# lyd405121/ti-raytrace

Measured on AMD Instinct MI355X. Metric: Mrays/s (primary+secondary) at 1024² 100k-tri, 1/2/4/8 GPU + HBM GB/s, higher is better.
Workload: dtype f32

## Files before the change

include/tirt.h:

```cpp
#ifndef TIRT_H
#define TIRT_H

#include <stdint.h>

#ifdef __cplusplus
extern "C" {
#endif

typedef struct tirt_ctx tirt_ctx;

#define TIRT_OK 0
#define TIRT_ERR_HIP (-1)
#define TIRT_ERR_ARG (-2)
#define TIRT_ERR_BUILD (-3)
#define TIRT_ERR_STACK (-4)

#define TIRT_TRAVERSE_ORDERED 0
#define TIRT_TRAVERSE_EXHAUSTIVE 1
#define TIRT_COUNT_NODES 2

typedef struct {
    uint64_t rays_closest;
    uint64_t rays_shadow;
    uint64_t box_closest;
// ... 92 lines not shown

int tirt_bvh_info(tirt_ctx *ctx, uint64_t out[4]);
int tirt_micro_gather_rate(tirt_ctx *ctx, uint64_t working_set_bytes, int iters, double *gbps_out);

int tirt_trace_timeline(tirt_ctx *ctx, uint64_t *out, int max_waves, int *n_waves);

int tirt_primary_beam_stats(tirt_ctx *ctx, uint64_t out[12]);

int tirt_stats(tirt_ctx *ctx, tirt_stats_t *out);
int tirt_stats_reset(tirt_ctx *ctx);

int tirt_kat_math(tirt_ctx *ctx, int fn, const float *x, const float *y, float *out, int n);
int tirt_kat_brdf(tirt_ctx *ctx, int which, const float *in, int in_stride, float *out, int out_stride, int n);
int tirt_kat_spec(tirt_ctx *ctx, int which, const float *in, int in_stride, float *out, int out_stride, int n);

typedef struct tirt_obj tirt_obj;
int tirt_obj_load(const char *path, tirt_obj **out);
void tirt_obj_free(tirt_obj *obj);
int tirt_obj_material_count(const tirt_obj *obj);
int tirt_obj_material_info(const tirt_obj *obj, int index, char *name, int name_cap, double *params, int *vertex_format,
                           int *is_default, long long *n_floats);
int tirt_obj_material_vertices(const tirt_obj *obj, int index, double *out, long long n_floats);

#ifdef __cplusplus
}
#endif
#endif
```

ti_raytrace_amd/_native.py:

```python
import ctypes as C
import os

import numpy as np

_HERE = os.path.dirname(os.path.abspath(__file__))
LIB_PATH = os.environ.get("TIRT_LIB_PATH") or os.path.join(_HERE, "csrc", "libtirt.so")

_f32p = np.ctypeslib.ndpointer(dtype=np.float32, flags="C_CONTIGUOUS")
_i32p = np.ctypeslib.ndpointer(dtype=np.int32, flags="C_CONTIGUOUS")


class TirtError(RuntimeError):
    pass


class TirtStackOverflow(TirtError):

    def __init__(self, msg, stats):
        TirtError.__init__(self, msg)
        self.stats = stats


ERR_STACK = -4

# ... 56 lines not shown
    "tirt_trace_shadow": (C.c_int, [_vp, _f32p, C.c_int, C.c_int, C.c_int, _f32p, _i32p, _vp]),
    "tirt_query_closest": (C.c_int, [_vp, _vp, C.c_int64, C.c_int64, C.c_int, C.c_int, _vp, _vp, _vp, C.c_int64, _vp, _vp]),
    "tirt_query_occluded": (C.c_int, [_vp, _vp, C.c_int64, C.c_int64, _vp, C.c_int64, C.c_float, C.c_int, C.c_int, _vp, _vp]),
    "tirt_comm_init": (C.c_int, [C.POINTER(_vp), C.c_int]),
    "tirt_film_reduce": (C.c_int, [C.POINTER(_vp), C.c_int, C.c_int]),
    "tirt_comm_destroy": (C.c_int, [C.POINTER(_vp), C.c_int]),
    "tirt_bvh_info": (C.c_int, [_vp, C.POINTER(C.c_uint64)]),
    "tirt_micro_gather_rate": (C.c_int, [_vp, C.c_uint64, C.c_int, C.POINTER(C.c_double)]),
    "tirt_trace_timeline": (C.c_int, [_vp, C.POINTER(C.c_uint64), C.c_int, C.POINTER(C.c_int)]),
    "tirt_primary_beam_stats": (C.c_int, [_vp, C.POINTER(C.c_uint64)]),
    "tirt_stats": (C.c_int, [_vp, C.POINTER(Stats)]),
    "tirt_stats_reset": (C.c_int, [_vp]),
    "tirt_kat_math": (C.c_int, [_vp, C.c_int, _f32p, _f32p, _f32p, C.c_int]),
    "tirt_kat_brdf": (C.c_int, [_vp, C.c_int, _f32p, C.c_int, _f32p, C.c_int, C.c_int]),
    "tirt_kat_spec": (C.c_int, [_vp, C.c_int, _f32p, C.c_int, _f32p, C.c_int, C.c_int]),
    "tirt_obj_load": (C.c_int, [C.c_char_p, C.POINTER(_vp)]),
    "tirt_obj_free": (None, [_vp]),
    "tirt_obj_material_count": (C.c_int, [_vp]),
    "tirt_obj_material_info": (C.c_int, [_vp, C.c_int, C.c_char_p, C.c_int, C.POINTER(C.c_double), C.POINTER(C.c_int),
                                         C.POINTER(C.c_int), C.POINTER(C.c_longlong)]),
    "tirt_obj_material_vertices": (C.c_int, [_vp, C.c_int, np.ctypeslib.ndpointer(dtype=np.float64, flags="C_CONTIGUOUS"), C.c_longlong]),
}

class SpectralTables(C.Structure):
    _fields_ = [("sensor", C.c_void_p), ("n_sensor", C.c_int), ("s_min", C.c_float), ("s_max", C.c_float), ("s_range", C.c_float),
                ("spd", C.c_void_p), ("spd_n", C.c_int * 4), ("spd_min", C.c_float * 4), ("spd_max", C.c_float * 4), ("spd_range", C.c_float * 4),
                ("tbl_scale", C.c_void_p), ("tbl_data", C.c_void_p), ("tbl_res", C.c_int),
                ("sky_cfg", C.c_void_p), ("sky_rad", C.c_void_p), ("sun_dir", C.c_float * 3)]


# ... 282 lines not shown

    def kat_math(self, fn, x, y=None):
        x = np.ascontiguousarray(x, np.float32)
        y = np.ascontiguousarray(y if y is not None else np.zeros_like(x), np.float32)
        out = np.zeros_like(x)
        check(lib().tirt_kat_math(self.handle, int(fn), x, y, out, x.size))
        return out

    def kat_brdf(self, which, inp, out_stride):
        inp = np.ascontiguousarray(inp, np.float32)
        n, stride = inp.shape
        out = np.zeros((n, out_stride), np.float32)
        check(lib().tirt_kat_brdf(self.handle, int(which), inp.reshape(-1), stride, out.reshape(-1), out_stride, n))
        return out

    def kat_spec(self, which, inp, out_stride):
        inp = np.ascontiguousarray(inp, np.float32)
        n, stride = inp.shape
        out = np.zeros((n, out_stride), np.float32)
        check(lib().tirt_kat_spec(self.handle, int(which), inp.reshape(-1), stride, out.reshape(-1), out_stride, n))
        return out


def device_count():
    v = C.c_int(0)
    check(lib().tirt_device_count(C.byref(v)))
    return v.value


class Communicator:
# ... 14 lines not shown
```

ti_raytrace_amd/csrc/tirt_api.hip:

```cpp
#include "tirt_internal.h"
#include "tirt_spectral.h"
#include <stddef.h>
#include <mutex>
#include <string.h>

namespace tirt {

static thread_local std::string g_error;
void set_error(const std::string &msg) { g_error = msg; }

SceneView scene_view(const tirt_ctx *c)
{
    SceneView s;
    s.vertex = c->vertex.as<float>(); s.primitive = c->primitive.as<int>(); s.material = c->material.as<float>();
    s.shape = c->shape.as<float>(); s.light = c->light.as<int>(); s.env = c->env.as<int>();
    s.mat_lrgb = c->mat_lrgb.as<float>(); s.shade_rec = c->shade_rec.as<float4>();
    s.n = c->n; s.light_count = c->light_count; s.env_w = c->env_w; s.env_h = c->env_h; s.env_power = c->env_power;
    return s;
}
BvhView bvh_view(const tirt_ctx *c)
{
    BvhView b;
    b.wnode = c->wnode.as<float4>(); b.tri = c->tri.as<float4>();
    b.cnode = c->cnode.as<uint4>(); b.top_count = c->wide_nodes + c->n_far_nodes < TR_TOP_SLOTS ? c->wide_nodes + c->n_far_nodes : TR_TOP_SLOTS; b.compact = c->compact.as<float>(); b.cparent = c->cparent.as<int>();
    for (int k = 0; k < 3; k++) { b.grid_min[k] = c->grid_min[k]; b.cell[k] = c->grid_cell[k]; b.inv_cell[k] = c->grid_inv_cell[k]; b.inv_extent[k] = c->grid_inv_extent[k]; }
    for (int k = 0; k < 3; k++) { b.root_min[k] = c->root_min[k]; b.root_max[k] = c->root_max[k]; }
    b.root_code = c->root_code;
    b.root_qcode = c->root_code;
    b.far_qcode = c->n_far_nodes ? c->wide_nodes : c->root_code;
    return b;
}
// ... 31 lines not shown
}
static int refresh_material_table(tirt_ctx *c)
{
    if (c->mat_lrgb.ensure(sizeof(float) * 3 * (size_t)c->nm)) return TIRT_ERR_HIP;
    hipLaunchKernelGGL(k_material_lrgb, dim3((c->nm + 63) / 64), dim3(64), 0, c->stream, c->material.as<float>(), c->nm, c->mat_lrgb.as<float>());
    return 0;
}

__global__ void k_shade_records(SceneView s, float4 *rec)
{
    const int i = blockIdx.x * blockDim.x + threadIdx.x;
    if (i >= s.n) return;
    const int *pr = s.primitive + (size_t)i * PRI_VEC;
    float4 *r = rec + (size_t)i * 8;
    const float mat = __int_as_float(pr[2]);
    if (pr[0] == PRIMITIVE_TRI) {
        const v3 v1 = vtx_pos(s, pr[1]), v2 = vtx_pos(s, pr[1] + 1), v3_ = vtx_pos(s, pr[1] + 2);
        const v3 n1 = vtx_nor(s, pr[1]), n2 = vtx_nor(s, pr[1] + 1), n3 = vtx_nor(s, pr[1] + 2);
        r[0] = make_float4(v1.x, v1.y, v1.z, mat); r[1] = make_float4(v2.x, v2.y, v2.z, __int_as_float(PRIMITIVE_TRI));
        r[2] = make_float4(v3_.x, v3_.y, v3_.z, 0.0f);
        r[3] = make_float4(n1.x, n1.y, n1.z, 0.0f); r[4] = make_float4(n2.x, n2.y, n2.z, 0.0f); r[5] = make_float4(n3.x, n3.y, n3.z, 0.0f);
    } else {
        const float *sh = s.shape + (size_t)pr[1] * SHA_VEC;
        r[0] = make_float4(sh[1], sh[2], sh[3], mat); r[1] = make_float4(sh[4], sh[0], 0.0f, __int_as_float(2));
        r[2] = r[3] = r[4] = r[5] = make_float4(0.0f, 0.0f, 0.0f, 0.0f);
    }
    r[6] = r[7] = make_float4(0.0f, 0.0f, 0.0f, 0.0f);
}
int ensure_shade_records(tirt_ctx *c)
{
    if (c->shade_rec_valid && c->shade_rec.p) return 0;
    if (c->shade_rec.ensure(sizeof(float4) * 8 * (size_t)c->n)) return TIRT_ERR_HIP;
    hipLaunchKernelGGL(k_shade_records, dim3((c->n + 255) / 256), dim3(256), 0, c->stream, scene_view(c), c->shade_rec.as<float4>());
    c->shade_rec_valid = true;
    return 0;
}

__global__ void k_total_area(SceneView s, int count, float *out)
{
    if (blockIdx.x == 0 && threadIdx.x == 0) {
        float a = 0.0f;
        for (int i = 0; i < count; i++) a += get_prim_area(s, s.light[i]);
        *out = a;
    }
}

__global__ void k_smooth_normal(SceneView s, int nv, const float *compact, const int *vertex_index, float *smooth)
{
    int i = blockIdx.x * blockDim.x + threadIdx.x;
// ... 116 lines not shown
        o[0] = schlick_fresnel(a[0]);
    } else if (which == 16) {
        float fb; v3 r = glass_sample_lambda(V(a[0], a[1], a[2]), V(a[3], a[4], a[5]), a[6], a[7], fb); o[0] = r.x; o[1] = r.y; o[2] = r.z; o[3] = fb;
    } else if (which == 17) {
        CameraView cv; for (int k = 0; k < 12; k++) cv.view_inv[k] = a[k];
        cv.eye[0] = cv.eye[1] = cv.eye[2] = 0.0f; cv.fx = a[16]; cv.fy = a[17]; cv.cx = a[18]; cv.cy = a[19];
        v3 r = camera_ray_direction(cv, (int)a[20], (int)a[21], a[22], a[23]); o[0] = r.x; o[1] = r.y; o[2] = r.z;
    } else if (which == 18) {
        const RayCtx r = make_ray(V(a[0], a[1], a[2]), V(a[3], a[4], a[5])); float tn;
        const int full = slabs(r, a[6], a[7], a[8], a[9], a[10], a[11], tn);
        o[0] = (float)full;
        o[1] = ray_has_parallel_axis(r) ? (float)full : (float)slabs_fast(r, a[6], a[7], a[8], a[9], a[10], a[11], tn);
    }
}

TD uint32_t mg_mix(uint32_t x) { x ^= x >> 16; x *= 0x7feb352du; x ^= x >> 15; x *= 0x846ca68bu; x ^= x >> 16; return x; }
__global__ __launch_bounds__(256) void k_micro_gather(const float4 *rec, uint32_t nrec, int iters, float *out)
{
    uint32_t s = mg_mix(blockIdx.x * 256 + threadIdx.x + 1);
    float acc = 0.0f;
    for (int it = 0; it < iters; it++) {
        s = mg_mix(s + it);
        const uint32_t idx = (uint32_t)(((unsigned long long)s * nrec) >> 32);
        const float4 *p = rec + (size_t)idx * 4;
        const float4 a = p[0], b = p[1], c = p[2], d = p[3];
        acc += a.x + b.y + c.z + d.w;
    }
    out[blockIdx.x * 256 + threadIdx.x] = acc;
}

// ... 55 lines not shown
    if (hipDeviceGetAttribute(&cus, hipDeviceAttributeMultiprocessorCount, device_id) == hipSuccess && cus > 0) {
        const int g = 5 * cus < 2048 ? 5 * cus : 2048;
        c->tr_grid = g; c->tr_grid_alone = g; c->cu_count = cus;
    } else (void)hipGetLastError();
    *out = c;
    return TIRT_OK;
}

void tirt_destroy(tirt_ctx *c)
{
    if (!c) return;
    if (c->comm) { tirt_ctx *one[1] = {c}; (void)tirt_comm_destroy(one, 1); }
    (void)hipSetDevice(c->device);
    (void)sync_all(c);
    drain_render_events(c);
    DevBuf *bufs[] = {&c->vertex, &c->primitive, &c->material, &c->shape, &c->light, &c->env, &c->mat_lrgb, &c->shade_rec, &c->morton_unsorted, &c->keys_a,
                      &c->keys_b, &c->vals_a, &c->vals_b, &c->hist, &c->morton_sorted, &c->bvh_node, &c->compact, &c->parent,
                      &c->flag, &c->subtree, &c->build_status, &c->leaf_compact, &c->wnode, &c->tri, &c->prim_slot, &c->cnode, &c->cparent, &c->csize, &c->wide_queue, &c->wide_levels, &c->sah_compact, &c->sah_csize, &c->sah_parent, &c->wide_dp, &c->sah_box, &c->sah_idx, &c->sah_tasks, &c->sah_counts, &c->hdr, &c->rgb,
                      &c->counters_mem, &c->spill, &c->trace_stage, &c->debug_mem, &c->query_mem, &c->dev_counters, &c->bdpt_px, &c->timeline, &c->pvb_set[0].count, &c->pvb_set[0].cand, &c->pvb_set[0].bound, &c->pvb_set[1].count, &c->pvb_set[1].cand, &c->pvb_set[1].bound, &c->pvb_stat, &c->pvb_tmp};
    for (DevBuf *b : bufs) b->release();
    for (auto &bl : c->bd) {
        DevBuf *bb[] = {&bl.items, &bl.state, &bl.rays, &bl.hits, &bl.qidx, &bl.ctr, &bl.rad};
        for (DevBuf *b : bb) b->release();
        if (bl.delta_done) (void)hipEventDestroy(bl.delta_done);
        if (bl.film_done) (void)hipEventDestroy(bl.film_done);
    }
    for (Lane &L : c->lanes) {
        DevBuf *lb[] = {&L.path_mem, &L.counters_mem, &L.spill};
        for (DevBuf *b : lb) b->release();
        if (L.film_done) (void)hipEventDestroy(L.film_done);
        if (L.stream) (void)hipStreamDestroy(L.stream);
// ... 105 lines not shown
        TIRT_REQUIRE(pr[2] >= 0 && pr[2] < nm, "tirt_scene_upload: material index out of range");
    }
    for (int i = 0; i < nl; i++) TIRT_REQUIRE(light[i] >= 0 && light[i] < n, "tirt_scene_upload: light index out of range");
    c->sphere_prims.clear();
    for (int i = 0; i < n; i++) {
        const int32_t *pr = primitive + (size_t)i * 3;
        if (pr[0] != PRIMITIVE_TRI && (int)shape[(size_t)pr[1] * 10] == SHAPE_SPHERE) c->sphere_prims.push_back(i);
    }
    hipStream_t st = c->stream;
    c->built = false;
    if (upload(c->vertex, vertex, sizeof(float) * 9 * (size_t)nv, st)) return TIRT_ERR_HIP;
    if (upload(c->primitive, primitive, sizeof(int) * 3 * (size_t)n, st)) return TIRT_ERR_HIP;
    if (upload(c->material, material, sizeof(float) * 10 * (size_t)nm, st)) return TIRT_ERR_HIP;
    if (upload(c->shape, shape, sizeof(float) * 10 * (size_t)ns, st)) return TIRT_ERR_HIP;
    if (upload(c->light, light, sizeof(int) * (size_t)nl, st)) return TIRT_ERR_HIP;
    c->nv = nv; c->n = n; c->nm = nm; c->ns = ns; c->nl = nl; c->light_count = light_count; c->shade_rec_valid = false;
    for (int k = 0; k < 3; k++) { c->bmin[k] = bmin[k]; c->bmax[k] = bmax[k]; }
    if (refresh_material_table(c)) return TIRT_ERR_HIP;
    if (!c->env.p) {
        int32_t z = 0;
        if (upload(c->env, &z, sizeof(int32_t), st)) return TIRT_ERR_HIP;
        c->env_w = 1; c->env_h = 1; c->env_power = 0.0f;
    }
    TIRT_HIP(hipStreamSynchronize(st));
    return TIRT_OK;
}

int tirt_material_upload(tirt_ctx *c, const float *material, int nm)
{
    CTX(c);
    if (sync_all(c)) return TIRT_ERR_HIP;
    TIRT_REQUIRE(material && nm == c->nm, "tirt_material_upload: material count differs from the uploaded scene");
    if (upload(c->material, material, sizeof(float) * 10 * (size_t)nm, c->stream)) return TIRT_ERR_HIP;
    if (refresh_material_table(c)) return TIRT_ERR_HIP;
    TIRT_HIP(hipStreamSynchronize(c->stream));
    return TIRT_OK;
}

int tirt_env_upload(tirt_ctx *c, const int32_t *rgb_packed, int w, int h, float power)
{
    CTX(c);
    if (sync_all(c)) return TIRT_ERR_HIP;
    TIRT_REQUIRE(rgb_packed && w >= 1 && h >= 1, "tirt_env_upload: bad image");
    if (upload(c->env, rgb_packed, sizeof(int32_t) * (size_t)w * h, c->stream)) return TIRT_ERR_HIP;
    c->env_w = w; c->env_h = h; c->env_power = power;
    TIRT_HIP(hipStreamSynchronize(c->stream));
    return TIRT_OK;
}

// ... 56 lines not shown
}

int tirt_process_normal(tirt_ctx *c, const int32_t *vertex_index)
{
    CTX(c);
    if (sync_all(c)) return TIRT_ERR_HIP;
    TIRT_REQUIRE(c->built && vertex_index, "tirt_process_normal: LBVH not built");
    if (c->nv == 0) return TIRT_OK;
    for (int i = 0; i < c->nv; i++) TIRT_REQUIRE(vertex_index[i] >= 0 && vertex_index[i] < c->n, "tirt_process_normal: vertex_index out of range");
    DevBuf vi, smooth;
    if (upload(vi, vertex_index, sizeof(int) * (size_t)c->nv, c->stream)) return TIRT_ERR_HIP;
    if (smooth.ensure(sizeof(float) * 3 * (size_t)c->nv)) { vi.release(); return TIRT_ERR_HIP; }
    const int B = 128, G = (c->nv + B - 1) / B;
    hipLaunchKernelGGL(k_smooth_normal, dim3(G), dim3(B), 0, c->stream, scene_view(c), c->nv, c->compact.as<float>(), vi.as<int>(), smooth.as<float>());
    hipLaunchKernelGGL(k_write_normal, dim3(G), dim3(B), 0, c->stream, c->vertex.as<float>(), c->nv, smooth.as<float>());
    c->shade_rec_valid = false;
    hipError_t e = hipStreamSynchronize(c->stream);
    vi.release(); smooth.release();
    TIRT_HIP(e);
    TIRT_HIP(hipGetLastError());
    return TIRT_OK;
}

int tirt_vertex_download(tirt_ctx *c, float *vertex)
{
    CTX(c);
    TIRT_REQUIRE(vertex, "tirt_vertex_download: null");
    TIRT_HIP(hipMemcpyAsync(vertex, c->vertex.p, sizeof(float) * 9 * (size_t)c->nv, hipMemcpyDeviceToHost, c->stream));
    TIRT_HIP(hipStreamSynchronize(c->stream));
    return TIRT_OK;
}
// ... 325 lines not shown
    TIRT_REQUIRE(in_stride >= need_in[which] && out_stride >= need_out[which], "tirt_kat_brdf: stride too small");
    if (n == 0) return TIRT_OK;
    DevBuf din, dout;
    int rc = TIRT_OK;
    if (upload(din, in, sizeof(float) * (size_t)n * in_stride, c->stream) || dout.ensure(sizeof(float) * (size_t)n * out_stride)) rc = TIRT_ERR_HIP;
    if (rc == TIRT_OK) {
        hipLaunchKernelGGL(k_kat_brdf, dim3((n + 255) / 256), dim3(256), 0, c->stream, which, din.as<float>(), in_stride, dout.as<float>(), out_stride, n);
        hipError_t e = hipMemcpyAsync(out, dout.p, sizeof(float) * (size_t)n * out_stride, hipMemcpyDeviceToHost, c->stream);
        if (e == hipSuccess) e = hipStreamSynchronize(c->stream);
        if (e != hipSuccess) { set_error(std::string("tirt_kat_brdf: ") + hipGetErrorString(e)); rc = TIRT_ERR_HIP; }
    }
    din.release(); dout.release();
    return rc;
}

}
```

ti_raytrace_amd/csrc/tirt_device.h:

```cpp
#pragma once
#include <hip/hip_runtime.h>
#include "tirt_math.h"

#define TD __device__ __forceinline__

namespace tirt {

constexpr int MAT_VEC = 10, VER_VEC = 9, PRI_VEC = 3, SHA_VEC = 10, NOD_VEC = 11, CPN_VEC = 9;
constexpr int SHAPE_SPHERE = 1, SHAPE_SPOT = 3, SHAPE_LASER = 4;
constexpr int PRIMITIVE_TRI = 1;
constexpr int MAT_DISNEY = 0, MAT_GLASS = 1, MAT_LIGHT = 2;
constexpr float INF_VALUE = 1000000.0f;
constexpr float PI_UF = (float)3.1415956;
constexpr float PI_SCENE = (float)3.1415926;

struct v3 { float x, y, z; };
TD v3 V(float x, float y, float z) { v3 r; r.x = x; r.y = y; r.z = z; return r; }
TD v3 operator+(v3 a, v3 b) { return V(a.x + b.x, a.y + b.y, a.z + b.z); }
TD v3 operator-(v3 a, v3 b) { return V(a.x - b.x, a.y - b.y, a.z - b.z); }
TD v3 operator*(v3 a, v3 b) { return V(a.x * b.x, a.y * b.y, a.z * b.z); }
TD v3 operator*(v3 a, float s) { return V(a.x * s, a.y * s, a.z * s); }
TD v3 operator/(v3 a, float s) { return V(a.x / s, a.y / s, a.z / s); }
TD v3 operator-(v3 a) { return V(-a.x, -a.y, -a.z); }
TD float dot(v3 a, v3 b) { return (a.x * b.x + a.y * b.y) + a.z * b.z; }
// ... 5 lines not shown
TD float maxf(float a, float b) { return a > b ? a : b; }
TD float clampf(float x, float lo, float hi) { return minf(hi, maxf(lo, x)); }
TD float signf(float x) { return x > 0.0f ? 1.0f : (x < 0.0f ? -1.0f : 0.0f); }
TD float mixf(float a, float b, float t) { return a * (1.0f - t) + b * t; }
TD v3 mix3(v3 a, v3 b, float t) { return V(mixf(a.x, b.x, t), mixf(a.y, b.y, t), mixf(a.z, b.z, t)); }

struct SceneView {
    const float *vertex;
    const int *primitive;
    const float *material;
    const float *shape;
    const int *light;
    const int *env;
    const float *mat_lrgb;
    const float4 *shade_rec;
    int n, light_count, env_w, env_h;
    float env_power;
};
struct CameraView { float view_inv[12]; float eye[3]; float fx, fy, cx, cy; };

TD v3 vtx_pos(const SceneView &s, int i) { const float *p = s.vertex + (size_t)i * VER_VEC; return V(p[0], p[1], p[2]); }
TD v3 vtx_nor(const SceneView &s, int i) { const float *p = s.vertex + (size_t)i * VER_VEC; return V(p[3], p[4], p[5]); }
TD v3 vtx_uv(const SceneView &s, int i)  { const float *p = s.vertex + (size_t)i * VER_VEC; return V(p[6], p[7], p[8]); }

struct RayCtx { float ox, oy, oz, dx, dy, dz, idx, idy, idz; };
TD RayCtx make_ray(v3 o, v3 d)
{
    RayCtx r; r.ox = o.x; r.oy = o.y; r.oz = o.z; r.dx = d.x; r.dy = d.y; r.dz = d.z;
    r.idx = 1.0f / d.x; r.idy = 1.0f / d.y; r.idz = 1.0f / d.z;
    return r;
// ... 64 lines not shown
    v3 oc = centre - origin;
    float dis_oc_square = dot(oc, oc);
    float dis_op = dot(direction, oc);
    float dis_cp = tm_sqrt(dis_oc_square - dis_op * dis_op);
    c_out = 0.0f;
    if (dis_cp < r) {
        float a = dot(direction, direction);
        float b = -2.0f * dis_op;
        float c = dis_oc_square - r * r;
        hit_t = (-b - tm_sqrt(b * b - 4.0f * a * c)) / 2.0f / a;
        c_out = c;
    }
    return hit_t;
}

struct HitAttr { v3 pos, gnor, nor, tex; };
TD HitAttr hit_attributes(const SceneView &s, v3 origin, v3 direction, int prim, float t, float u, float v)
{
    HitAttr h; h.pos = h.gnor = h.nor = h.tex = V(0.0f, 0.0f, 0.0f);
    const int *pr = s.primitive + (size_t)prim * PRI_VEC;
    v3 gn = V(0.0f, 0.0f, 0.0f), nn = gn;
    if (pr[0] == PRIMITIVE_TRI) {
        int vi = pr[1];
        float a = 1.0f - u - v, b = u, c = v;
        v3 v1 = vtx_pos(s, vi), v2 = vtx_pos(s, vi + 1), v3_ = vtx_pos(s, vi + 2);
        v3 n1 = vtx_nor(s, vi), n2 = vtx_nor(s, vi + 1), n3 = vtx_nor(s, vi + 2);
        v3 t1 = vtx_uv(s, vi), t2 = vtx_uv(s, vi + 1), t3 = vtx_uv(s, vi + 2);
        v3 v13 = v3_ - v1, v12 = v2 - v1;
        gn = cross(v12, v13);
        h.pos = (v1 * a + v2 * b) + v3_ * c;
        h.tex = (t1 * a + t2 * b) + t3 * c;
        nn = (n1 * a + n2 * b) + n3 * c;
    } else {
        const float *sh = s.shape + (size_t)pr[1] * SHA_VEC;
// ... 3 lines not shown
            h.pos = origin + direction * t;
            nn = V(h.pos.x - c, h.pos.y - c, h.pos.z - c);
            gn = nn;
        }
    }
    h.gnor = normalized(gn); h.nor = normalized(nn);
    return h;
}

TD HitAttr hit_attributes_rec(const float4 *rec, v3 origin, v3 direction, int prim, float t, float u, float v, int &mat_id)
{
    HitAttr h; h.pos = h.gnor = h.nor = h.tex = V(0.0f, 0.0f, 0.0f);
    const float4 *r = rec + (size_t)prim * 8;
    const float4 r0 = r[0], r1 = r[1];
    mat_id = __float_as_int(r0.w);
    v3 gn = V(0.0f, 0.0f, 0.0f), nn = gn;
    if (__float_as_int(r1.w) == PRIMITIVE_TRI) {
        const float4 r2 = r[2], r3 = r[3], r4 = r[4], r5 = r[5];
        float a = 1.0f - u - v, b = u, c = v;
        v3 v1 = V(r0.x, r0.y, r0.z), v2 = V(r1.x, r1.y, r1.z), v3_ = V(r2.x, r2.y, r2.z);
        v3 n1 = V(r3.x, r3.y, r3.z), n2 = V(r4.x, r4.y, r4.z), n3 = V(r5.x, r5.y, r5.z);
        v3 v13 = v3_ - v1, v12 = v2 - v1;
        gn = cross(v12, v13);
        h.pos = (v1 * a + v2 * b) + v3_ * c;
        nn = (n1 * a + n2 * b) + n3 * c;
    } else if ((int)r1.y == SHAPE_SPHERE) {
        float c;
        (void)intersect_sphere(origin, direction, V(r0.x, r0.y, r0.z), r1.x, c);
        h.pos = origin + direction * t;
        nn = V(h.pos.x - c, h.pos.y - c, h.pos.z - c);
        gn = nn;
    }
    h.gnor = normalized(gn); h.nor = normalized(nn);
    return h;
}

TD float srgb_to_lrgb1(float c) { return (c < 0.04045f) ? c / 12.92f : tm_pow((c + 0.055f) / 1.055f, 2.4f); }
TD v3 srgb_to_lrgb(v3 c) { return V(srgb_to_lrgb1(c.x), srgb_to_lrgb1(c.y), srgb_to_lrgb1(c.z)); }
TD float lrgb_to_srgb1(float c)
{
    const float e = (float)(1.0 / 2.4);
    float o = (c < 0.0031308f) ? c * 12.92f : 1.055f * tm_pow(c, e) - 0.055f;
    return clampf(o, 0.0f, 1.0f);
}
TD float tone_aces1(float x)
{
    const float a = 2.51f, b = 0.03f, c = 2.43f, d = 0.59f, e = 0.14f;
    return clampf((x * (a * x + b)) / (x * (c * x + d) + e), 0.0f, 1.0f);
// ... 186 lines not shown
        if (st == SHAPE_SPOT) {
            const float NdotL = absf(dot(light_dir, light_normal));
            const float x1 = sh[4], x2 = sh[5];
            const float x = tm_acos(NdotL);
            if (x > x2) visable = 0.0f;
            else if (x > x1) visable *= 1.0f - (x - x1) / (x2 - x1);
        } else if (st == SHAPE_LASER) {
            choice_pdf = 1.0f / (float)s.light_count;
            const float proj = dot(light_dir, light_normal) * light_dist;
            const float r = tm_sqrt(light_dist * light_dist - proj * proj);
            if (r > sh[4]) visable = 0.0f;
        }
    }
    return visable;
}
TD void map_to_disk(float u1, float u2, float &r, float &phi)
{
    phi = 0.0f; r = 0.0f;
    const float a = 2.0f * u1 - 1.0f, b = 2.0f * u2 - 1.0f;
    if (a > -b) {
        if (a > b) { r = a; phi = (PI_UF / 4.0f) * (b / a); }
        else { r = b; phi = (PI_UF / 4.0f) * (2.0f - a / b); }
    } else {
        if (a < b) { r = -a; phi = (PI_UF / 4.0f) * (4.0f + b / a); }
        else { r = -b; phi = (b == 0.0f) ? 0.0f : (PI_UF / 4.0f) * (6.0f - a / b); }
    }
}
TD float get_prim_angle(const SceneView &s, int index, v3 v)
{
    float ret = 0.0f;
// ... 46 lines not shown
```

ti_raytrace_amd/csrc/tirt_internal.h:

```cpp
#pragma once
#include <hip/hip_runtime.h>
#include <stdint.h>
#include <stdio.h>
#include <string>
#include <vector>
#include "../../include/tirt.h"
#include "tirt_device.h"

namespace tirt {

void set_error(const std::string &msg);

#define TIRT_HIP(call)                                                                          \
    do {                                                                                        \
        hipError_t e__ = (call);                                                                \
        if (e__ != hipSuccess) {                                                                \
            tirt::set_error(std::string(#call) + ": " + hipGetErrorString(e__));                \
            return TIRT_ERR_HIP;                                                                \
        }                                                                                       \
    } while (0)

#define TIRT_REQUIRE(cond, msg)                                                                 \
    do {                                                                                        \
        if (!(cond)) { tirt::set_error(msg); return TIRT_ERR_ARG; }                             \
// ... 156 lines not shown
    hipEvent_t film_done = nullptr; bool film_recorded = false;
    size_t path_capacity = 0;
    DevBuf path_mem, counters_mem, spill;
    PathState ps;
};

}

struct tirt_ctx {
    int device = 0;
    hipStream_t stream = nullptr;
    hipEvent_t ev0 = nullptr, ev1 = nullptr;

    int nv = 0, n = 0, nm = 0, ns = 0, nl = 0, light_count = 0;
    float bmin[3] = {0, 0, 0}, bmax[3] = {0, 0, 0};
    tirt::DevBuf vertex, primitive, material, shape, light, env, mat_lrgb, shade_rec;
    bool shade_rec_valid = false;
    int env_w = 0, env_h = 0; float env_power = 0.0f;

    bool built = false;
    tirt::DevBuf morton_unsorted;
    tirt::DevBuf keys_a, keys_b, vals_a, vals_b;
    tirt::DevBuf hist;
    tirt::DevBuf morton_sorted;
    tirt::DevBuf bvh_node, compact;
    tirt::DevBuf parent, flag, subtree, build_status, leaf_compact;
    tirt::DevBuf wnode, tri, prim_slot;
    tirt::DevBuf cnode, cparent, csize, wide_queue, wide_levels;
    int wide_nodes = 0;
    tirt::DevBuf sah_compact, sah_csize, sah_parent, wide_dp, sah_box, sah_idx, sah_tasks, sah_counts;
    int use_sah = 1, sah_levels = 0, built_sah = 0;
    std::vector<int> sphere_prims;
// ... 134 lines not shown
```

ti_raytrace_amd/csrc/tirt_render.hip:

```cpp
#include "tirt_internal.h"
#include "tirt_spectral.h"

namespace tirt {

constexpr int TR_GRID_MAX = 2048;

enum { KIND_CLOSEST = 0, KIND_SHADOW_ACC = 1, KIND_MIXED = 2, KIND_QUERY = 3 };
#if !defined(TIRT_EXPERIMENTS) && (defined(TR_PAD) || defined(TR_PADG))
#error "the bound ladder (TR_PAD / TR_PADG) needs an experiments build: add -DTIRT_EXPERIMENTS"
#endif
struct TraceArgs {
    BvhView bvh;
    const float *ox, *oy, *oz, *dx, *dy, *dz;
    float eye[3];
    const int *count_ptr; int count_fixed;
    float4 *hit;
    const int *sprim, *sdst; const float *sdist, *scr, *scg, *scb; float *rr, *rg, *rb, *fr, *fg, *fb;
    const float *scw; float *rw, *fw;
    int *spill; int spill_depth;
    const float *sox, *soy, *soz, *sdx, *sdy, *sdz; const int *scount_ptr;
    int *fetch; int slice_log2;
    int slices_contig;
    int lds_depth;
    int refill_min;
// ... 20 lines not shown
    const float t = hrec.x;
    if (t < INF_VALUE) {
        const int prim_id = __float_as_int(hrec.w);
        int mat_id;
        const HitAttr h = hit_attributes_rec(sc.shade_rec, origin, direction, prim_id, t, hrec.y, hrec.z, mat_id);
        const v3 normal = h.nor;
        const v3 fnormal = normal * signf(dot(-direction, h.gnor));
        const float *m = sc.material + (size_t)mat_id * MAT_VEC;
        const v3 mat_color = V(m[2], m[3], m[4]);
        const int mat_type = (int)m[0];
        if (mat_type == MAT_LIGHT) {
            const float fCosTheta = absf(dot(direction, h.gnor));
            if (perfect_spec == 1) {
                radiance = radiance + throughout * mat_color;
            } else {
                const float area = get_prim_area(sc, prim_id) * (float)sc.light_count;
                const float light_pdf = (t * t) / (area * fCosTheta);
                radiance = radiance + (throughout * power_heuristic(brdf_pdf, light_pdf)) * mat_color;
            }
        } else {
            s.shaded = true;
            const v3 reflect_color = V(sc.mat_lrgb[mat_id * 3], sc.mat_lrgb[mat_id * 3 + 1], sc.mat_lrgb[mat_id * 3 + 2]);
            v3 next_dir; float f_or_b = 1.0f, brdf = 1.0f;
            if (mat_type == MAT_GLASS) {
                perfect_spec = 1;
                next_dir = glass_sample(m, direction, normal, tm_rand(seed, pixel, frame, dim0 + TM_SLOT_GLASS), f_or_b);
                brdf = 1.0f; brdf_pdf = 1.0f;
            } else {
                perfect_spec = 0;
                if (sc.light_count > 0) {
                int lidx = (int)(tm_rand(seed, pixel, frame, dim0 + TM_SLOT_LIGHT) * (float)sc.light_count);
                if (lidx >= sc.light_count) lidx = sc.light_count - 1;
                const int light_prim = sc.light[lidx];
                const float ra = tm_rand(seed, pixel, frame, dim0 + TM_SLOT_LA);
                const float rb = tm_rand(seed, pixel, frame, dim0 + TM_SLOT_LB);
                v3 light_pos, light_normal;
                get_prim_random_point_normal(sc, light_prim, ra, rb, light_pos, light_normal);
                const int lmat = sc.primitive[(size_t)light_prim * PRI_VEC + 2];
                const float *lm = sc.material + (size_t)lmat * MAT_VEC;
                const v3 light_emission0 = V(lm[2], lm[3], lm[4]);
                const float light_area = get_prim_area(sc, light_prim);
                float light_choice_pdf = 1.0f / ((float)sc.light_count * light_area);
                light_normal = normalized(light_normal);
                v3 light_dir = h.pos - light_pos;
                const float light_dist = norm(light_dir);
                light_dir = light_dir / light_dist;
                const v3 light_emission = light_emission0 * light_shape_visible(sc, light_prim, light_dir, light_normal, light_dist, light_choice_pdf);
                const float NdotL_surface = dot(fnormal, light_dir);
                const float NdotL_light = dot(light_normal, light_dir);
                if ((NdotL_surface < 0.0f) & (NdotL_light > 0.0f)) {
                    s.want_shadow = true;
                    float e_pdf;
                    const float e_brdf = disney_evaluate_pdf(m, fnormal, -direction, -light_dir, e_pdf);
                    const float light_pdf = light_dist * light_dist * light_choice_pdf / NdotL_light;
                    v3 c = V(0.0f, 0.0f, 0.0f);
                    int expect = -2;
                    if (e_pdf > 0.0f) {
                        const float w = power_heuristic(light_pdf, e_pdf) / maxf(0.0001f, light_pdf);
                        c = light_emission * w;
                        c = c * throughout;
                        c = c * reflect_color;
                        c = c * e_brdf;
// ... 766 lines not shown
                if (mat_type == MAT_LIGHT) {
                    const float fCosTheta = dot(direction, normal);
                    if (fCosTheta < 0.0f) radiance = radiance + ((throughout * light_rad) * light_tint);
                } else {
                    n_shaded++;
                    const f4s reflect_spec = get_spec_power(sp, m, Lambda);
                    v3 next_dir; float f_or_b = 1.0f, brdf = 1.0f, brdf_pdf = 1.0f;
                    if (mat_type == MAT_GLASS) {
                        const int index = (int)(tm_rand(seed, pixel, frame, dim0 + TM_SLOT_HERO) * (float)HERO_N);
                        const float rnd_lambda = Lambda + (float)index * HERO_LAMBDA_STEP;
                        next_dir = glass_sample_lambda(direction, normal, rnd_lambda, tm_rand(seed, pixel, frame, dim0 + TM_SLOT_GLASS), f_or_b);
                    } else {
                        if (sc.light_count > 0) {
                            int lidx = (int)(tm_rand(seed, pixel, frame, dim0 + TM_SLOT_LIGHT) * (float)sc.light_count);
                            if (lidx >= sc.light_count) lidx = sc.light_count - 1;
                            const int light_prim = sc.light[lidx];
                            const float ra = tm_rand(seed, pixel, frame, dim0 + TM_SLOT_LA);
                            const float rb = tm_rand(seed, pixel, frame, dim0 + TM_SLOT_LB);
                            v3 light_pos, light_normal;
                            get_prim_random_point_normal(sc, light_prim, ra, rb, light_pos, light_normal);
                            const float light_area = get_prim_area(sc, light_prim);
                            float light_choice_pdf = 1.0f / ((float)sc.light_count * light_area);
                            light_normal = normalized(light_normal);
                            v3 light_dir = h.pos - light_pos;
                            const float light_dist = norm(light_dir);
                            light_dir = light_dir / light_dist;
                            (void)light_shape_visible(sc, light_prim, light_dir, light_normal, light_dist, light_choice_pdf);
                            const float NdotL_surface = dot(fnormal, light_dir);
                            const float NdotL_light = dot(light_normal, light_dir);
                            if ((NdotL_surface < 0.0f) & (NdotL_light > 0.0f)) {
                                want_shadow = true;
                                float e_pdf;
                                const float e_brdf = disney_evaluate_pdf(m, fnormal, -direction, -light_dir, e_pdf);
                                const float light_pdf = light_dist * light_dist * light_choice_pdf / NdotL_light;
                                f4s c = f4_set(0.0f);
                                int expect = -2;
                                if (e_pdf > 0.0f) {
                                    const float w = power_heuristic(light_pdf, e_pdf) / maxf(0.0001f, light_pdf);
                                    c = light_rad * w;
                                    c = c * light_tint;
                                    c = c * throughout;
                                    c = c * reflect_spec;
// ... 319 lines not shown
```

Before: 5562.

## Precompute per-light sample records and per-primitive geometric normal/area for shading

```diff
diff --git a/include/tirt.h b/include/tirt.h
--- a/include/tirt.h
+++ b/include/tirt.h
@@ -130,6 +130,9 @@
 int tirt_kat_brdf(tirt_ctx *ctx, int which, const float *in, int in_stride, float *out, int out_stride, int n);
 int tirt_kat_spec(tirt_ctx *ctx, int which, const float *in, int in_stride, float *out, int out_stride, int n);
 
+int tirt_shade_table_download(tirt_ctx *ctx, int which, float *out, uint64_t floats);
+int tirt_kat_shade_tables(tirt_ctx *ctx, int which, const float *in, float *out, int n);
+
 typedef struct tirt_obj tirt_obj;
 int tirt_obj_load(const char *path, tirt_obj **out);
 void tirt_obj_free(tirt_obj *obj);
diff --git a/ti_raytrace_amd/_native.py b/ti_raytrace_amd/_native.py
--- a/ti_raytrace_amd/_native.py
+++ b/ti_raytrace_amd/_native.py
@@ -94,6 +94,8 @@
     "tirt_kat_math": (C.c_int, [_vp, C.c_int, _f32p, _f32p, _f32p, C.c_int]),
     "tirt_kat_brdf": (C.c_int, [_vp, C.c_int, _f32p, C.c_int, _f32p, C.c_int, C.c_int]),
     "tirt_kat_spec": (C.c_int, [_vp, C.c_int, _f32p, C.c_int, _f32p, C.c_int, C.c_int]),
+    "tirt_shade_table_download": (C.c_int, [_vp, C.c_int, _f32p, C.c_uint64]),
+    "tirt_kat_shade_tables": (C.c_int, [_vp, C.c_int, _vp, _f32p, C.c_int]),
     "tirt_obj_load": (C.c_int, [C.c_char_p, C.POINTER(_vp)]),
     "tirt_obj_free": (None, [_vp]),
     "tirt_obj_material_count": (C.c_int, [_vp]),
@@ -406,6 +408,19 @@
         check(lib().tirt_kat_brdf(self.handle, int(which), inp.reshape(-1), stride, out.reshape(-1), out_stride, n))
         return out
 
+    def shade_table_download(self, which, count):
+        out = np.zeros((int(count), 8, 4), np.float32)
+        check(lib().tirt_shade_table_download(self.handle, int(which), out.reshape(-1), out.size))
+        return out
+
+    def kat_shade_tables(self, which, n, inp=None):
+        if inp is not None:
+            inp = np.ascontiguousarray(inp, np.float32)
+            n = inp.shape[0]
+        out = np.zeros((int(n), 4) if which == 0 else (int(n), 5) if which == 1 else (int(n), 2, 12), np.float32)
+        check(lib().tirt_kat_shade_tables(self.handle, int(which), _ptr(inp), out.reshape(-1), int(n)))
+        return out
+
     def kat_spec(self, which, inp, out_stride):
         inp = np.ascontiguousarray(inp, np.float32)
         n, stride = inp.shape
diff --git a/ti_raytrace_amd/csrc/tirt_api.hip b/ti_raytrace_amd/csrc/tirt_api.hip
--- a/ti_raytrace_amd/csrc/tirt_api.hip
+++ b/ti_raytrace_amd/csrc/tirt_api.hip
@@ -14,7 +14,7 @@
     SceneView s;
     s.vertex = c->vertex.as<float>(); s.primitive = c->primitive.as<int>(); s.material = c->material.as<float>();
     s.shape = c->shape.as<float>(); s.light = c->light.as<int>(); s.env = c->env.as<int>();
-    s.mat_lrgb = c->mat_lrgb.as<float>(); s.shade_rec = c->shade_rec.as<float4>();
+    s.mat_lrgb = c->mat_lrgb.as<float>(); s.shade_rec = c->shade_rec.as<float4>(); s.light_rec = c->light_rec.as<float4>();
     s.n = c->n; s.light_count = c->light_count; s.env_w = c->env_w; s.env_h = c->env_h; s.env_power = c->env_power;
     return s;
 }
@@ -76,25 +76,66 @@
     const int *pr = s.primitive + (size_t)i * PRI_VEC;
     float4 *r = rec + (size_t)i * 8;
     const float mat = __int_as_float(pr[2]);
+    const float area = get_prim_area(s, i);
+    r[6] = r[7] = make_float4(0.0f, 0.0f, 0.0f, 0.0f);
     if (pr[0] == PRIMITIVE_TRI) {
         const v3 v1 = vtx_pos(s, pr[1]), v2 = vtx_pos(s, pr[1] + 1), v3_ = vtx_pos(s, pr[1] + 2);
         const v3 n1 = vtx_nor(s, pr[1]), n2 = vtx_nor(s, pr[1] + 1), n3 = vtx_nor(s, pr[1] + 2);
+        const v3 v13 = v3_ - v1, v12 = v2 - v1;
+        const v3 gnor = normalized(cross(v12, v13));
         r[0] = make_float4(v1.x, v1.y, v1.z, mat); r[1] = make_float4(v2.x, v2.y, v2.z, __int_as_float(PRIMITIVE_TRI));
         r[2] = make_float4(v3_.x, v3_.y, v3_.z, 0.0f);
         r[3] = make_float4(n1.x, n1.y, n1.z, 0.0f); r[4] = make_float4(n2.x, n2.y, n2.z, 0.0f); r[5] = make_float4(n3.x, n3.y, n3.z, 0.0f);
+        r[6] = make_float4(gnor.x, gnor.y, gnor.z, area);
     } else {
         const float *sh = s.shape + (size_t)pr[1] * SHA_VEC;
-        r[0] = make_float4(sh[1], sh[2], sh[3], mat); r[1] = make_float4(sh[4], sh[0], 0.0f, __int_as_float(2));
+        r[0] = make_float4(sh[1], sh[2], sh[3], mat); r[1] = make_float4(sh[4], sh[0], area, __int_as_float(2));
         r[2] = r[3] = r[4] = r[5] = make_float4(0.0f, 0.0f, 0.0f, 0.0f);
     }
+}
+__global__ void k_light_records(SceneView s, float4 *rec)
+{
+    const int i = blockIdx.x * blockDim.x + threadIdx.x;
+    if (i >= s.light_count) return;
+    const int light_prim = s.light[i];
+    const int *pr = s.primitive + (size_t)light_prim * PRI_VEC;
+    float4 *r = rec + (size_t)i * LIGHT_REC_QUADS;
+    const float *lm = s.material + (size_t)pr[2] * MAT_VEC;
+    const v3 em = V(lm[2], lm[3], lm[4]);
+    const float light_area = get_prim_area(s, light_prim);
+    float light_choice_pdf = 1.0f / ((float)s.light_count * light_area);
+    if (pr[0] == PRIMITIVE_TRI) {
+        const v3 v1 = vtx_pos(s, pr[1]), v2 = vtx_pos(s, pr[1] + 1), v3_ = vtx_pos(s, pr[1] + 2);
+        const v3 n1 = vtx_nor(s, pr[1]), n2 = vtx_nor(s, pr[1] + 1), n3 = vtx_nor(s, pr[1] + 2);
+        const v3 e31 = v3_ - v1, e21 = v2 - v1;
+        r[0] = make_float4(v1.x, v1.y, v1.z, light_area); r[1] = make_float4(e31.x, e31.y, e31.z, light_choice_pdf);
+        r[2] = make_float4(e21.x, e21.y, e21.z, __int_as_float(-1));
+        r[3] = make_float4(n1.x, n1.y, n1.z, em.x); r[4] = make_float4(n2.x, n2.y, n2.z, em.y); r[5] = make_float4(n3.x, n3.y, n3.z, em.z);
+    } else {
+        const float *sh = s.shape + (size_t)pr[1] * SHA_VEC;
+        int st = (int)sh[0];
+        if (st == SHAPE_LASER) light_choice_pdf = 1.0f / (float)s.light_count;
+        if (st == -1) st = -2;
+        r[0] = make_float4(sh[1], sh[2], sh[3], light_area); r[1] = make_float4(sh[4], sh[5], 0.0f, light_choice_pdf);
+        r[2] = make_float4(0.0f, 0.0f, 0.0f, __int_as_float(st));
+        r[3] = make_float4(sh[7], sh[8], sh[9], em.x); r[4] = make_float4(0.0f, 0.0f, 0.0f, em.y); r[5] = make_float4(0.0f, 0.0f, 0.0f, em.z);
+    }
     r[6] = r[7] = make_float4(0.0f, 0.0f, 0.0f, 0.0f);
 }
 int ensure_shade_records(tirt_ctx *c)
 {
-    if (c->shade_rec_valid && c->shade_rec.p) return 0;
-    if (c->shade_rec.ensure(sizeof(float4) * 8 * (size_t)c->n)) return TIRT_ERR_HIP;
-    hipLaunchKernelGGL(k_shade_records, dim3((c->n + 255) / 256), dim3(256), 0, c->stream, scene_view(c), c->shade_rec.as<float4>());
-    c->shade_rec_valid = true;
+    if (!(c->shade_rec_valid && c->shade_rec.p)) {
+        if (c->shade_rec.ensure(sizeof(float4) * 8 * (size_t)c->n)) return TIRT_ERR_HIP;
+        hipLaunchKernelGGL(k_shade_records, dim3((c->n + 255) / 256), dim3(256), 0, c->stream, scene_view(c), c->shade_rec.as<float4>());
+        c->shade_rec_valid = true;
+    }
+    if (!(c->light_rec_valid && c->light_rec.p)) {
+        const int nl = c->light_count > 0 ? c->light_count : 1;
+        if (c->light_rec.ensure(sizeof(float4) * LIGHT_REC_QUADS * (size_t)nl)) return TIRT_ERR_HIP;
+        if (c->light_count > 0)
+            hipLaunchKernelGGL(k_light_records, dim3((c->light_count + 63) / 64), dim3(64), 0, c->stream, scene_view(c), c->light_rec.as<float4>());
+        c->light_rec_valid = true;
+    }
     return 0;
 }
 
@@ -241,6 +282,63 @@
     }
 }
 
+__global__ void k_kat_shade_tables(SceneView s, int which, float *out, int n)
+{
+    const int i = blockIdx.x * blockDim.x + threadIdx.x;
+    if (i >= n) return;
+    if (which == 0) {
+        float *o = out + (size_t)i * 4;
+        v3 g = V(0.0f, 0.0f, 0.0f);
+        if (s.primitive[(size_t)i * PRI_VEC] == PRIMITIVE_TRI) g = hit_attributes(s, g, V(0.0f, 0.0f, 1.0f), i, 1.0f, 0.25f, 0.25f).gnor;
+        o[0] = g.x; o[1] = g.y; o[2] = g.z; o[3] = get_prim_area(s, i);
+    } else {
+        float *o = out + (size_t)i * 5;
+        const int light_prim = s.light[i];
+        const float *lm = s.material + (size_t)s.primitive[(size_t)light_prim * PRI_VEC + 2] * MAT_VEC;
+        const float light_area = get_prim_area(s, light_prim);
+        float light_choice_pdf = 1.0f / ((float)s.light_count * light_area);
+        (void)light_shape_visible(s, light_prim, V(0.0f, 0.0f, 1.0f), V(0.0f, 0.0f, 1.0f), 1.0f, light_choice_pdf);
+        o[0] = light_area; o[1] = light_choice_pdf; o[2] = lm[2]; o[3] = lm[3]; o[4] = lm[4];
+    }
+}
+TD void kat_nee_store(float *o, v3 pos, v3 nor, v3 em, float area, float pdf, float dist)
+{ o[0] = pos.x; o[1] = pos.y; o[2] = pos.z; o[3] = nor.x; o[4] = nor.y; o[5] = nor.z; o[6] = em.x; o[7] = em.y; o[8] = em.z; o[9] = area; o[10] = pdf; o[11] = dist; }
+__global__ void k_kat_light_sample(SceneView s, const float *in, float *out, int n)
+{
+    const int i = blockIdx.x * blockDim.x + threadIdx.x;
+    if (i >= n) return;
+    const float *a = in + (size_t)i * 6;
+    float *o = out + (size_t)i * 24;
+    int lidx = (int)(a[0] * (float)s.light_count);
+    if (lidx >= s.light_count) lidx = s.light_count - 1;
+    if (lidx < 0) lidx = 0;
+    const v3 p = V(a[3], a[4], a[5]);
+    {
+        const int light_prim = s.light[lidx];
+        v3 light_pos, light_normal;
+        get_prim_random_point_normal(s, light_prim, a[1], a[2], light_pos, light_normal);
+        const float *lm = s.material + (size_t)s.primitive[(size_t)light_prim * PRI_VEC + 2] * MAT_VEC;
+        const float light_area = get_prim_area(s, light_prim);
+        float light_choice_pdf = 1.0f / ((float)s.light_count * light_area);
+        light_normal = normalized(light_normal);
+        v3 light_dir = p - light_pos;
+        const float light_dist = norm(light_dir);
+        light_dir = light_dir / light_dist;
+        const v3 em = V(lm[2], lm[3], lm[4]) * light_shape_visible(s, light_prim, light_dir, light_normal, light_dist, light_choice_pdf);
+        kat_nee_store(o, light_pos, light_normal, em, light_area, light_choice_pdf, light_dist);
+    }
+    {
+        v3 light_pos, light_normal;
+        const LightRec lr = light_sample_rec(s.light_rec, lidx, a[1], a[2], light_pos, light_normal);
+        light_normal = normalized(light_normal);
+        v3 light_dir = p - light_pos;
+        const float light_dist = norm(light_dir);
+        light_dir = light_dir / light_dist;
+        const v3 em = lr.emission * light_shape_visible_rec(lr, light_dir, light_normal, light_dist);
+        kat_nee_store(o + 12, light_pos, light_normal, em, lr.area, lr.choice_pdf, light_dist);
+    }
+}
+
 TD uint32_t mg_mix(uint32_t x) { x ^= x >> 16; x *= 0x7feb352du; x ^= x >> 15; x *= 0x846ca68bu; x ^= x >> 16; return x; }
 __global__ __launch_bounds__(256) void k_micro_gather(const float4 *rec, uint32_t nrec, int iters, float *out)
 {
@@ -326,7 +424,7 @@
     (void)hipSetDevice(c->device);
     (void)sync_all(c);
     drain_render_events(c);
-    DevBuf *bufs[] = {&c->vertex, &c->primitive, &c->material, &c->shape, &c->light, &c->env, &c->mat_lrgb, &c->shade_rec, &c->morton_unsorted, &c->keys_a,
+    DevBuf *bufs[] = {&c->vertex, &c->primitive, &c->material, &c->shape, &c->light, &c->env, &c->mat_lrgb, &c->shade_rec, &c->light_rec, &c->morton_unsorted, &c->keys_a,
                       &c->keys_b, &c->vals_a, &c->vals_b, &c->hist, &c->morton_sorted, &c->bvh_node, &c->compact, &c->parent,
                       &c->flag, &c->subtree, &c->build_status, &c->leaf_compact, &c->wnode, &c->tri, &c->prim_slot, &c->cnode, &c->cparent, &c->csize, &c->wide_queue, &c->wide_levels, &c->sah_compact, &c->sah_csize, &c->sah_parent, &c->wide_dp, &c->sah_box, &c->sah_idx, &c->sah_tasks, &c->sah_counts, &c->hdr, &c->rgb,
                       &c->counters_mem, &c->spill, &c->trace_stage, &c->debug_mem, &c->query_mem, &c->dev_counters, &c->bdpt_px, &c->timeline, &c->pvb_set[0].count, &c->pvb_set[0].cand, &c->pvb_set[0].bound, &c->pvb_set[1].count, &c->pvb_set[1].cand, &c->pvb_set[1].bound, &c->pvb_stat, &c->pvb_tmp};
@@ -462,7 +560,7 @@
     if (upload(c->material, material, sizeof(float) * 10 * (size_t)nm, st)) return TIRT_ERR_HIP;
     if (upload(c->shape, shape, sizeof(float) * 10 * (size_t)ns, st)) return TIRT_ERR_HIP;
     if (upload(c->light, light, sizeof(int) * (size_t)nl, st)) return TIRT_ERR_HIP;
-    c->nv = nv; c->n = n; c->nm = nm; c->ns = ns; c->nl = nl; c->light_count = light_count; c->shade_rec_valid = false;
+    c->nv = nv; c->n = n; c->nm = nm; c->ns = ns; c->nl = nl; c->light_count = light_count; c->shade_rec_valid = false; c->light_rec_valid = false;
     for (int k = 0; k < 3; k++) { c->bmin[k] = bmin[k]; c->bmax[k] = bmax[k]; }
     if (refresh_material_table(c)) return TIRT_ERR_HIP;
     if (!c->env.p) {
@@ -481,6 +579,7 @@
     TIRT_REQUIRE(material && nm == c->nm, "tirt_material_upload: material count differs from the uploaded scene");
     if (upload(c->material, material, sizeof(float) * 10 * (size_t)nm, c->stream)) return TIRT_ERR_HIP;
     if (refresh_material_table(c)) return TIRT_ERR_HIP;
+    c->light_rec_valid = false;
     TIRT_HIP(hipStreamSynchronize(c->stream));
     return TIRT_OK;
 }
@@ -567,7 +666,7 @@
     const int B = 128, G = (c->nv + B - 1) / B;
     hipLaunchKernelGGL(k_smooth_normal, dim3(G), dim3(B), 0, c->stream, scene_view(c), c->nv, c->compact.as<float>(), vi.as<int>(), smooth.as<float>());
     hipLaunchKernelGGL(k_write_normal, dim3(G), dim3(B), 0, c->stream, c->vertex.as<float>(), c->nv, smooth.as<float>());
-    c->shade_rec_valid = false;
+    c->shade_rec_valid = false; c->light_rec_valid = false;
     hipError_t e = hipStreamSynchronize(c->stream);
     vi.release(); smooth.release();
     TIRT_HIP(e);
@@ -923,4 +1022,42 @@
     return rc;
 }
 
-}
+int tirt_shade_table_download(tirt_ctx *c, int which, float *out, uint64_t floats)
+{
+    CTX(c);
+    TIRT_REQUIRE(out && (which == 0 || which == 1), "tirt_shade_table_download: bad args");
+    TIRT_REQUIRE(c->n >= 1, "tirt_shade_table_download: no scene");
+    if (sync_all(c)) return TIRT_ERR_HIP;
+    if (ensure_shade_records(c)) return TIRT_ERR_HIP;
+    const uint64_t have = which == 0 ? (uint64_t)32 * c->n : (uint64_t)4 * LIGHT_REC_QUADS * c->light_count;
+    TIRT_REQUIRE(floats == have, "tirt_shade_table_download: 32 floats per primitive (which 0) or per light (which 1)");
+    if (floats) TIRT_HIP(hipMemcpyAsync(out, which == 0 ? c->shade_rec.p : c->light_rec.p, sizeof(float) * floats, hipMemcpyDeviceToHost, c->stream));
+    TIRT_HIP(hipStreamSynchronize(c->stream));
+    return TIRT_OK;
+}
+
+int tirt_kat_shade_tables(tirt_ctx *c, int which, const float *in, float *out, int n)
+{
+    CTX(c);
+    TIRT_REQUIRE(out && n >= 0 && which >= 0 && which <= 2, "tirt_kat_shade_tables: bad args");
+    TIRT_REQUIRE(c->n >= 1, "tirt_kat_shade_tables: no scene");
+    TIRT_REQUIRE(which == 2 ? (in && c->light_count > 0) : n == (which == 0 ? c->n : c->light_count), "tirt_kat_shade_tables: n is the primitive / light count; which 2 needs input and a light");
+    if (n == 0) return TIRT_OK;
+    if (sync_all(c)) return TIRT_ERR_HIP;
+    if (ensure_shade_records(c)) return TIRT_ERR_HIP;
+    const size_t out_floats = (size_t)n * (which == 0 ? 4 : which == 1 ? 5 : 24);
+    DevBuf din, dout;
+    int rc = TIRT_OK;
+    if ((which == 2 && upload(din, in, sizeof(float) * 6 * (size_t)n, c->stream)) || dout.ensure(sizeof(float) * out_floats)) rc = TIRT_ERR_HIP;
+    if (rc == TIRT_OK) {
+        if (which == 2) hipLaunchKernelGGL(k_kat_light_sample, dim3((n + 255) / 256), dim3(256), 0, c->stream, scene_view(c), din.as<float>(), dout.as<float>(), n);
+        else hipLaunchKernelGGL(k_kat_shade_tables, dim3((n + 255) / 256), dim3(256), 0, c->stream, scene_view(c), which, dout.as<float>(), n);
+        hipError_t e = hipMemcpyAsync(out, dout.p, sizeof(float) * out_floats, hipMemcpyDeviceToHost, c->stream);
+        if (e == hipSuccess) e = hipStreamSynchronize(c->stream);
+        if (e != hipSuccess) { set_error(std::string("tirt_kat_shade_tables: ") + hipGetErrorString(e)); rc = TIRT_ERR_HIP; }
+    }
+    din.release(); dout.release();
+    return rc;
+}
+
+}
diff --git a/ti_raytrace_amd/csrc/tirt_device.h b/ti_raytrace_amd/csrc/tirt_device.h
--- a/ti_raytrace_amd/csrc/tirt_device.h
+++ b/ti_raytrace_amd/csrc/tirt_device.h
@@ -43,6 +43,7 @@
     const int *env;
     const float *mat_lrgb;
     const float4 *shade_rec;
+    const float4 *light_rec;
     int n, light_count, env_w, env_h;
     float env_power;
 };
@@ -137,10 +138,10 @@
     return hit_t;
 }
 
-struct HitAttr { v3 pos, gnor, nor, tex; };
+struct HitAttr { v3 pos, gnor, nor, tex; float area; };
 TD HitAttr hit_attributes(const SceneView &s, v3 origin, v3 direction, int prim, float t, float u, float v)
 {
-    HitAttr h; h.pos = h.gnor = h.nor = h.tex = V(0.0f, 0.0f, 0.0f);
+    HitAttr h; h.pos = h.gnor = h.nor = h.tex = V(0.0f, 0.0f, 0.0f); h.area = 0.0f;
     const int *pr = s.primitive + (size_t)prim * PRI_VEC;
     v3 gn = V(0.0f, 0.0f, 0.0f), nn = gn;
     if (pr[0] == PRIMITIVE_TRI) {
@@ -174,14 +175,15 @@
     const float4 *r = rec + (size_t)prim * 8;
     const float4 r0 = r[0], r1 = r[1];
     mat_id = __float_as_int(r0.w);
-    v3 gn = V(0.0f, 0.0f, 0.0f), nn = gn;
-    if (__float_as_int(r1.w) == PRIMITIVE_TRI) {
-        const float4 r2 = r[2], r3 = r[3], r4 = r[4], r5 = r[5];
+    h.area = r1.z;
+    v3 nn = V(0.0f, 0.0f, 0.0f);
+    const bool tri = __float_as_int(r1.w) == PRIMITIVE_TRI;
+    if (tri) {
+        const float4 r2 = r[2], r3 = r[3], r4 = r[4], r5 = r[5], r6 = r[6];
         float a = 1.0f - u - v, b = u, c = v;
         v3 v1 = V(r0.x, r0.y, r0.z), v2 = V(r1.x, r1.y, r1.z), v3_ = V(r2.x, r2.y, r2.z);
         v3 n1 = V(r3.x, r3.y, r3.z), n2 = V(r4.x, r4.y, r4.z), n3 = V(r5.x, r5.y, r5.z);
-        v3 v13 = v3_ - v1, v12 = v2 - v1;
-        gn = cross(v12, v13);
+        h.gnor = V(r6.x, r6.y, r6.z); h.area = r6.w;
         h.pos = (v1 * a + v2 * b) + v3_ * c;
         nn = (n1 * a + n2 * b) + n3 * c;
     } else if ((int)r1.y == SHAPE_SPHERE) {
@@ -189,9 +191,9 @@
         (void)intersect_sphere(origin, direction, V(r0.x, r0.y, r0.z), r1.x, c);
         h.pos = origin + direction * t;
         nn = V(h.pos.x - c, h.pos.y - c, h.pos.z - c);
-        gn = nn;
-    }
-    h.gnor = normalized(gn); h.nor = normalized(nn);
+    }
+    h.nor = normalized(nn);
+    if (!tri) h.gnor = h.nor;
     return h;
 }
 
@@ -408,6 +410,46 @@
     }
     return visable;
 }
+constexpr int LIGHT_REC_QUADS = 8;
+struct LightRec { v3 emission; float area, choice_pdf, p0, p1; int kind; };
+TD LightRec light_sample_rec(const float4 *lrec, int lidx, float a, float b, v3 &pos, v3 &nor)
+{
+    const float4 *r = lrec + (size_t)lidx * LIGHT_REC_QUADS;
+    const float4 r0 = r[0], r1 = r[1], r2 = r[2], r3 = r[3], r4 = r[4], r5 = r[5];
+    LightRec L; L.emission = V(r3.w, r4.w, r5.w); L.area = r0.w; L.choice_pdf = r1.w; L.p0 = r1.x; L.p1 = r1.y; L.kind = __float_as_int(r2.w);
+    pos = V(0.0f, 0.0f, 0.0f); v3 normal = pos;
+    if (L.kind == -1) {
+        const v3 v1 = V(r0.x, r0.y, r0.z), e31 = V(r1.x, r1.y, r1.z), e21 = V(r2.x, r2.y, r2.z);
+        const v3 n1 = V(r3.x, r3.y, r3.z), n2 = V(r4.x, r4.y, r4.z), n3 = V(r5.x, r5.y, r5.z);
+        if (a + b > 1.0f) { a = 1.0f - a; b = 1.0f - b; }
+        pos = (v1 + e31 * a) + e21 * b;
+        normal = normalized((n1 * (1.0f - a - b) + n2 * a) + n3 * b);
+    } else if (L.kind == SHAPE_SPHERE) {
+        normal = uniform_sample_sphere(a, b);
+        pos = V(r0.x, r0.y, r0.z) + normal * L.p0;
+    } else if (L.kind == SHAPE_SPOT || L.kind == SHAPE_LASER) {
+        normal = V(r3.x, r3.y, r3.z);
+        pos = V(r0.x, r0.y, r0.z);
+    }
+    nor = normalized(normal);
+    return L;
+}
+TD float light_shape_visible_rec(const LightRec &L, v3 light_dir, v3 light_normal, float light_dist)
+{
+    float visable = 1.0f;
+    if (L.kind == SHAPE_SPOT) {
+        const float NdotL = absf(dot(light_dir, light_normal));
+        const float x1 = L.p0, x2 = L.p1;
+        const float x = tm_acos(NdotL);
+        if (x > x2) visable = 0.0f;
+        else if (x > x1) visable *= 1.0f - (x - x1) / (x2 - x1);
+    } else if (L.kind == SHAPE_LASER) {
+        const float proj = dot(light_dir, light_normal) * light_dist;
+        const float r = tm_sqrt(light_dist * light_dist - proj * proj);
+        if (r > L.p0) visable = 0.0f;
+    }
+    return visable;
+}
 TD void map_to_disk(float u1, float u2, float &r, float &phi)
 {
     phi = 0.0f; r = 0.0f;
diff --git a/ti_raytrace_amd/csrc/tirt_internal.h b/ti_raytrace_amd/csrc/tirt_internal.h
--- a/ti_raytrace_amd/csrc/tirt_internal.h
+++ b/ti_raytrace_amd/csrc/tirt_internal.h
@@ -194,8 +194,9 @@
 
     int nv = 0, n = 0, nm = 0, ns = 0, nl = 0, light_count = 0;
     float bmin[3] = {0, 0, 0}, bmax[3] = {0, 0, 0};
-    tirt::DevBuf vertex, primitive, material, shape, light, env, mat_lrgb, shade_rec;
+    tirt::DevBuf vertex, primitive, material, shape, light, env, mat_lrgb, shade_rec, light_rec;
     bool shade_rec_valid = false;
+    bool light_rec_valid = false;
     int env_w = 0, env_h = 0; float env_power = 0.0f;
 
     bool built = false;
diff --git a/ti_raytrace_amd/csrc/tirt_render.hip b/ti_raytrace_amd/csrc/tirt_render.hip
--- a/ti_raytrace_amd/csrc/tirt_render.hip
+++ b/ti_raytrace_amd/csrc/tirt_render.hip
@@ -58,7 +58,7 @@
             if (perfect_spec == 1) {
                 radiance = radiance + throughout * mat_color;
             } else {
-                const float area = get_prim_area(sc, prim_id) * (float)sc.light_count;
+                const float area = h.area * (float)sc.light_count;
                 const float light_pdf = (t * t) / (area * fCosTheta);
                 radiance = radiance + (throughout * power_heuristic(brdf_pdf, light_pdf)) * mat_color;
             }
@@ -75,21 +75,16 @@
                 if (sc.light_count > 0) {
                 int lidx = (int)(tm_rand(seed, pixel, frame, dim0 + TM_SLOT_LIGHT) * (float)sc.light_count);
                 if (lidx >= sc.light_count) lidx = sc.light_count - 1;
-                const int light_prim = sc.light[lidx];
                 const float ra = tm_rand(seed, pixel, frame, dim0 + TM_SLOT_LA);
                 const float rb = tm_rand(seed, pixel, frame, dim0 + TM_SLOT_LB);
                 v3 light_pos, light_normal;
-                get_prim_random_point_normal(sc, light_prim, ra, rb, light_pos, light_normal);
-                const int lmat = sc.primitive[(size_t)light_prim * PRI_VEC + 2];
-                const float *lm = sc.material + (size_t)lmat * MAT_VEC;
-                const v3 light_emission0 = V(lm[2], lm[3], lm[4]);
-                const float light_area = get_prim_area(sc, light_prim);
-                float light_choice_pdf = 1.0f / ((float)sc.light_count * light_area);
+                const LightRec lr = light_sample_rec(sc.light_rec, lidx, ra, rb, light_pos, light_normal);
+                const float light_choice_pdf = lr.choice_pdf;
                 light_normal = normalized(light_normal);
                 v3 light_dir = h.pos - light_pos;
                 const float light_dist = norm(light_dir);
                 light_dir = light_dir / light_dist;
-                const v3 light_emission = light_emission0 * light_shape_visible(sc, light_prim, light_dir, light_normal, light_dist, light_choice_pdf);
+                const v3 light_emission = lr.emission * light_shape_visible_rec(lr, light_dir, light_normal, light_dist);
                 const float NdotL_surface = dot(fnormal, light_dir);
                 const float NdotL_light = dot(light_normal, light_dir);
                 if ((NdotL_surface < 0.0f) & (NdotL_light > 0.0f)) {
@@ -886,18 +881,15 @@
                         if (sc.light_count > 0) {
                             int lidx = (int)(tm_rand(seed, pixel, frame, dim0 + TM_SLOT_LIGHT) * (float)sc.light_count);
                             if (lidx >= sc.light_count) lidx = sc.light_count - 1;
-                            const int light_prim = sc.light[lidx];
                             const float ra = tm_rand(seed, pixel, frame, dim0 + TM_SLOT_LA);
                             const float rb = tm_rand(seed, pixel, frame, dim0 + TM_SLOT_LB);
                             v3 light_pos, light_normal;
-                            get_prim_random_point_normal(sc, light_prim, ra, rb, light_pos, light_normal);
-                            const float light_area = get_prim_area(sc, light_prim);
-                            float light_choice_pdf = 1.0f / ((float)sc.light_count * light_area);
+                            const LightRec lr = light_sample_rec(sc.light_rec, lidx, ra, rb, light_pos, light_normal);
+                            const float light_choice_pdf = lr.choice_pdf;
                             light_normal = normalized(light_normal);
                             v3 light_dir = h.pos - light_pos;
                             const float light_dist = norm(light_dir);
                             light_dir = light_dir / light_dist;
-                            (void)light_shape_visible(sc, light_prim, light_dir, light_normal, light_dist, light_choice_pdf);
                             const float NdotL_surface = dot(fnormal, light_dir);
                             const float NdotL_light = dot(light_normal, light_dir);
                             if ((NdotL_surface < 0.0f) & (NdotL_light > 0.0f)) {
```

After: 5633 (median of 6 runs). 1.01x the previous value.
